# HBioquant/DiffBindFR

Hardware: AMD Instinct MI355X
Metric: poses_per_sec (higher is better)
Workload: dtype f32

## Files before the change

### diffbindfr_amd/build.py

```python
import os
import subprocess
import sys
from concurrent.futures import ThreadPoolExecutor

HERE = os.path.dirname(os.path.abspath(__file__))
CSRC = os.path.join(HERE, "csrc")
LIB = os.path.join(HERE, "libdbfr.so")
SOURCES = ["api.cpp", "so3_host.cpp", "conv.hip", "conv2.hip", "conv2h.hip", "convz.hip", "graph.hip", "heads.hip", "export.hip", "mdn.hip", "probe.hip", "vina.hip", "modes.hip", "posecheck.hip", "xtc.hip", "sites.hip", "interactions.hip", "pocketcheck.hip", "sasa.hip", "apoholo.hip", "hetero.hip"]
FLAGS = ["--offload-arch=gfx950", "-O3", "-std=c++17", "-fPIC", "-Wno-unused-result"]
if os.environ.get("DBFR_BUILD_DEV") == "1":
    FLAGS.append("-DDBFR_DEV_VARIANTS")
FILE_FLAGS = {"conv.hip": ["-ffp-contract=fast", "-fno-slp-vectorize", "-Wno-array-bounds"] + ([f"-DCONV_NB={os.environ['DBFR_BUILD_NB']}"] if "DBFR_BUILD_NB" in os.environ else [])
              + ([f"-DCONV_PRIO={os.environ['DBFR_BUILD_PRIO']}"] if "DBFR_BUILD_PRIO" in os.environ else [])
              + ([f"-DCONV_XPF={os.environ['DBFR_BUILD_XPF']}"] if "DBFR_BUILD_XPF" in os.environ else [])}
FILE_FLAGS["mdn.hip"] = ["-ffp-contract=off"]
FILE_FLAGS["conv2.hip"] = ["-ffp-contract=fast", "-fno-slp-vectorize", "-Wno-array-bounds"]
FILE_FLAGS["conv2h.hip"] = FILE_FLAGS["conv2.hip"] + ["-Rpass-analysis=kernel-resource-usage"]
FILE_FLAGS["convz.hip"] = FILE_FLAGS["conv2h.hip"]
DEFAULT_FP = ["-ffp-contract=off"]
FILE_FLAGS["vina.hip"] = DEFAULT_FP + ["-Rpass-analysis=kernel-resource-usage"]
FILE_FLAGS["modes.hip"] = FILE_FLAGS["vina.hip"]
FILE_FLAGS["posecheck.hip"] = FILE_FLAGS["vina.hip"]
FILE_FLAGS["xtc.hip"] = FILE_FLAGS["vina.hip"]
FILE_FLAGS["sites.hip"] = FILE_FLAGS["vina.hip"]
FILE_FLAGS["interactions.hip"] = FILE_FLAGS["vina.hip"]
FILE_FLAGS["pocketcheck.hip"] = FILE_FLAGS["vina.hip"]
FILE_FLAGS["sasa.hip"] = FILE_FLAGS["vina.hip"]
FILE_FLAGS["apoholo.hip"] = FILE_FLAGS["vina.hip"]
FILE_FLAGS["hetero.hip"] = FILE_FLAGS["vina.hip"]


def source_hash(dev=False):
    import hashlib
    h = hashlib.sha256()
    files = sorted([os.path.join(CSRC, f) for f in os.listdir(CSRC) if f.endswith((".cpp", ".hip", ".h", ".inc"))])
    files.append(os.path.join(HERE, "..", "include", "dbfr.h"))
    for f in files:
        h.update(os.path.basename(f).encode())
        h.update(open(f, "rb").read())
    if dev:
        h.update(b"DBFR_DEV_VARIANTS")
    return h.hexdigest()[:16]


def check_m0(hipcc, src):
    import re
    import tempfile
    with tempfile.TemporaryDirectory() as tmp:
        out = os.path.join(tmp, "convz.s")
        cmd = [hipcc, "-x", "hip", "-S", "--cuda-device-only", src, "-o", out] + [f for f in FLAGS + FILE_FLAGS["convz.hip"] if not f.startswith("-Rpass")]
        r = subprocess.run(cmd, capture_output=True, text=True)
        if r.returncode != 0:
            raise RuntimeError("hipcc -S failed (m0 check):\n" + r.stderr)
        lines = open(out).read().splitlines()
    ours = re.compile(r"^\s*s_mov_b32 m0, s\d+\s*$")
    bad = []
    for i, l in enumerate(lines):
        code = l.split(";")[0]
        if re.search(r"\bm0\b", code) and not ours.match(code):
            bad.append(f"{i + 1}: {l.strip()}")
        if ours.match(code) and not any("global_load_lds_dword" in x for x in lines[i + 1:i + 4]):
            bad.append(f"{i + 1}: s_mov_b32 m0 without an LDS-DMA load behind it: {l.strip()}")
    if bad:
        raise RuntimeError("convz.hip: the compiler (or an edit) uses m0 outside the LDS-DMA gathers -- the undeclared writes of prefetch_x are no longer safe:\n  " + "\n  ".join(bad[:10]))


def _stale(target, deps):
    if not os.path.exists(target):
        return True
    t = os.path.getmtime(target)
    return any(os.path.getmtime(d) > t for d in deps)


def build(force=False, verbose=True):
    hipcc = os.environ.get("HIPCC", "/opt/rocm/bin/hipcc")
    headers = [os.path.join(CSRC, "common.h"), os.path.join(CSRC, "frames.h"), os.path.join(CSRC, "residue_tables.inc"), os.path.join(HERE, "..", "include", "dbfr.h")]
    objs, jobs = [], []
    bid = source_hash(dev="-DDBFR_DEV_VARIANTS" in FLAGS)
    stamp = os.path.join(CSRC, ".build_id")
    if not os.path.exists(stamp) or open(stamp).read() != bid:
        open(stamp, "w").write(bid)
    headers.append(stamp)
# ... 29 lines not shown
```

### diffbindfr_amd/csrc/api.cpp

```cpp
#include <cmath>
#include <cstdio>
#include <cstring>
#include <algorithm>
#include <atomic>
#include <map>

#include "common.h"

void launch_conv(const ConvArgs& a, hipStream_t st);
void launch_conv_layer(const ConvArgs* c4, hipStream_t st);
void launch_conv2(const Conv2Args& a, hipStream_t st);
void launch_conv2h(const Conv2Args& a, hipStream_t st);
void launch_convz(const ConvZArgs& a, hipStream_t st);
void launch_reduce_ln(const float* msg, const int* row_start, const int* row_cnt, int N, int D, const LNDesc& ln,
                      const float* old, int D_old, float* out, int ldo, int mode, hipStream_t st, const uint8_t* first = nullptr, unsigned long long sc_lanes = 0);
struct ReduceLayerArgs {
  const float* msg[4]; const int* row_start[4]; const int* row_cnt[4]; LNDesc ln[4];
  int NL, NA, D, D_old;
  const float* old_l; const float* old_a; float* out_l; float* out_a;
  const uint8_t* first[4]; unsigned long long sc_lanes[4];
};
static unsigned long long convz_sc_lanes(const ConvZ& z) {
  unsigned long long m = 0;
  for (int i = 0; i < z.n_io; ++i) m |= 0xfffull << (z.out_off[i] / 4);
// ... 1633 lines not shown
  if (rc) return rc;
  if (!step || !scores || !z || !err_word_out) return fail(DBFR_ERR_ARG, "dbfr_test_sde_step: null argument");
  if (!scores->tr || !scores->rot || !z->z_tr || !z->z_rot || (b->NTOR > 0 && (!scores->tor || !z->z_tor)) ||
      (!m->cfg.no_sc_torsion && b->NSC > 0 && (!scores->sc_tor || !z->z_sc)))
    return fail(DBFR_ERR_ARG, "dbfr_test_sde_step: null score or noise array");
  hipStream_t st = (hipStream_t)hip_stream;
  HIPCHECK(hipMemsetAsync(err_word_out, 0, sizeof(int32_t), st));
  pose_update(m, b, *step, *scores, z->z_tr, z->z_rot, z->z_tor, z->z_sc, nullptr, atom14_out, nullptr, err_word_out, st);
  HIPCHECK(hipGetLastError());
  return DBFR_OK;
}

extern "C" int dbfr_test_chunk_table(const int32_t* tgt, const int32_t* n_edges_dev, int32_t max_edges, int32_t span, int32_t* scratch, int32_t cap,
                                     int32_t* chunk_es, int32_t* chunk_gl, void* hip_stream) {
  if (!tgt || !n_edges_dev || !scratch || !chunk_es || !chunk_gl || span <= 0 || max_edges < 0 || cap <= 0) return fail(DBFR_ERR_ARG, "dbfr_test_chunk_table: bad argument");
  g_launch_err = false;
  const int n_span = std::max((max_edges + span - 1) / span, 1);
  launch_flat_chunks(tgt, n_edges_dev, max_edges, span, n_span, scratch, cap, chunk_es, chunk_gl, (hipStream_t)hip_stream);
  HIPCHECK(hipGetLastError());
  return take_launch_error();
}

extern "C" int dbfr_test_conv(dbfr_model* m, int32_t layer, int32_t family, int32_t n_edges, const int32_t* n_edges_dev,
                              const int32_t* tgt, const int32_t* gth, const float* emb, const float* sh,
                              const float* tab1, int32_t ld1, const int32_t* idx1, const float* tab2, int32_t ld2,
                              const int32_t* idx2, const float* x, int32_t ldx, float* msg, void* hip_stream) {
  return test_conv_impl(m, false, layer, family, n_edges, n_edges_dev, tgt, gth, emb, sh, tab1, ld1, idx1, tab2, ld2, idx2, x, ldx,
                        msg, hip_stream);
}

extern "C" int dbfr_test_conv2(dbfr_model* m, int32_t layer, int32_t family, int32_t n_edges, const int32_t* n_edges_dev,
                               const int32_t* tgt, const int32_t* gth, const float* emb, const float* sh,
                               const float* tab1, int32_t ld1, const int32_t* idx1, const float* tab2, int32_t ld2,
                               const int32_t* idx2, const float* x, int32_t ldx, float* msg, void* hip_stream) {
  return test_conv_impl(m, true, layer, family, n_edges, n_edges_dev, tgt, gth, emb, sh, tab1, ld1, idx1, tab2, ld2, idx2, x, ldx,
                        msg, hip_stream);
}

extern "C" int dbfr_test_reduce_ln2(dbfr_model* m, int32_t layer, int32_t family, const float* msg, const int32_t* row_start, const int32_t* row_cnt,
                                    int32_t n_nodes, const float* old, int32_t d_old, float* out, int32_t mode, const uint8_t* seg_first, void* hip_stream) {
  if (!m) return fail(DBFR_ERR_ARG, "null model");
  const ConvW* cw = pick_conv(m, layer, family);
  if (!cw) return fail(DBFR_ERR_ARG, "no such conv");
  unsigned long long lanes = 0;
  if (seg_first) {
    if (layer == -1 || cw->K != 144) return fail(DBFR_ERR_ARG, "dbfr_test_reduce_ln2: seg_first with a conv that has no reduce-first form");
    lanes = convz_sc_lanes(layer >= 0 ? m->layerz[layer][family] : layer == -2 ? m->tor_convz : m->sc_convz);
  }
  launch_reduce_ln(msg, row_start, row_cnt, n_nodes, cw->D_out, cw->ln, old, d_old, out, cw->D_out, mode, (hipStream_t)hip_stream, seg_first, lanes);
  HIPCHECK(hipGetLastError());
  return DBFR_OK;
}

extern "C" int dbfr_test_reduce_ln(dbfr_model* m, int32_t layer, int32_t family, const float* msg,
                                   const int32_t* row_start, const int32_t* row_cnt, int32_t n_nodes, const float* old,
                                   int32_t d_old, float* out, int32_t mode, void* hip_stream) {
  if (!m) return fail(DBFR_ERR_ARG, "null model");
  const ConvW* cw = pick_conv(m, layer, family);
  if (!cw) return fail(DBFR_ERR_ARG, "no such conv");
  launch_reduce_ln(msg, row_start, row_cnt, n_nodes, cw->D_out, cw->ln, old, d_old, out, cw->D_out, mode,
                   (hipStream_t)hip_stream);
  HIPCHECK(hipGetLastError());
  return DBFR_OK;
}
```

### diffbindfr_amd/csrc/conv.hip

```cpp
#include <cstdio>
#include <cstdlib>
#include <type_traits>
#include <vector>

#include "common.h"

#ifndef CONV_PRIO
#define CONV_PRIO 0
#endif
#ifndef CONV_XPF
#define CONV_XPF 0
#endif
#ifndef CONV_NB2_WAVES
#define CONV_NB2_WAVES 2
#endif
#define XS_LD (MAXD + 4)

typedef float f32x4 __attribute__((ext_vector_type(4)));

#define TRACE_BLOCKS 1024
#define TRACE_TILES 48
#define TRACE_REC (2 + 3 * TRACE_TILES + 8)
#define RSTAMP(k) do { if ((ABL & 16) && a.trace && bid < TRACE_BLOCKS && lane == 0) a.trace[((size_t)bid * 4 + wave) * TRACE_REC + 2 + 3 * TRACE_TILES + (k)] = __builtin_amdgcn_s_memrealtime(); } while (0)
#define TSTAMP(k) do { if ((ABL & 16) && a.trace && bid < TRACE_BLOCKS && lane == 0) a.trace[((size_t)bid * 4 + wave) * TRACE_REC + 2 + 3 * TRACE_TILES + (k)] = __builtin_readcyclecounter(); } while (0)
// ... 462 lines not shown
  for (int bk = 0; bk < ln.nblk; ++bk) {
    const int mul = ln.mul[bk], dim = ln.dim[bk], off = ln.off[bk];
    const int nel = mul * dim;
    float mean[3] = {0.f, 0.f, 0.f};
    for (int i = lane; i < nel; i += 64) {
      int comp = i % dim;
      float v = buf[wave][off + i];
      if (comp == 0) mean[0] += v; else if (comp == 1) mean[1] += v; else mean[2] += v;
    }
#pragma unroll
    for (int c = 0; c < 3; ++c) {
      for (int o = 32; o > 0; o >>= 1) mean[c] += __shfl_xor(mean[c], o);
      mean[c] /= (float)mul;
    }
    float sq = 0.f;
    for (int i = lane; i < nel; i += 64) {
      int u = i / dim, comp = i - u * dim;
      float v = buf[wave][off + i] - (comp == 0 ? mean[0] : comp == 1 ? mean[1] : mean[2]) * ln.mean_shift[iw + u];
      buf[wave][off + i] = v;
      sq += v * v;
    }
    __syncthreads();
    for (int o = 32; o > 0; o >>= 1) sq += __shfl_xor(sq, o);
    const float inv = 1.0f / sqrtf(sq / (float)nel + 1e-5f);
    for (int i = lane; i < nel; i += 64) {
      int u = i / dim;
      float v = buf[wave][off + i] * (inv * ln.weight[iw + u]);
      if (ln.is0e[bk]) v += ln.bias[ib + u];
      buf[wave][off + i] = v;
    }
    iw += mul;
    if (ln.is0e[bk]) ib += mul;
  }
  __syncthreads();
#pragma unroll
  for (int j = 0; j < 3; ++j) {
    int c = lane + 64 * j;
    if (c < D && live) {
      float v = buf[wave][c];
      float* o = out + (size_t)node * ldo + c;
      if (mode == 0) v = (c < D_old ? old[(size_t)node * D_old + c] : 0.f) + v;
      else if (mode == 1) v = *o + v;
      *o = v;
    }
  }
}

void launch_reduce_ln(const float* msg, const int* row_start, const int* row_cnt, int N, int D, const LNDesc& ln,
                      const float* old, int D_old, float* out, int ldo, int mode, hipStream_t st, const uint8_t* first, unsigned long long sc_lanes) {
  if (N <= 0) return;
  hipLaunchKernelGGL(k_reduce_ln, dim3((N + 3) / 4), dim3(256), 0, st, msg, row_start, row_cnt, N, D, ln, old, D_old,
                     out, ldo, mode, first, sc_lanes);
}

struct ReduceLayerArgs {
  const float* msg[4]; const int* row_start[4]; const int* row_cnt[4]; LNDesc ln[4];
  int NL, NA, D, D_old;
  const float* old_l; const float* old_a; float* out_l; float* out_a;
  const uint8_t* first[4]; unsigned long long sc_lanes[4];
};

__device__ __forceinline__ void mean_ln(const float* __restrict__ msg, int rs, int rc, int D, const LNDesc& ln, float* bw, int lane, const uint8_t* first, unsigned long long sc_lanes) {
  const int d4 = D >> 2;
  const f32x4 acc = row_sum(msg, rs, rc, D, lane, first, sc_lanes);
  if (lane < d4) {
    const float cntf = (float)max(rc, 1);
    bw[4 * lane] = acc[0] / cntf; bw[4 * lane + 1] = acc[1] / cntf; bw[4 * lane + 2] = acc[2] / cntf; bw[4 * lane + 3] = acc[3] / cntf;
  }
  __builtin_amdgcn_wave_barrier();
  int iw = 0, ib = 0;
  for (int bk = 0; bk < ln.nblk; ++bk) {
    const int mul = ln.mul[bk], dim = ln.dim[bk], off = ln.off[bk];
    const int nel = mul * dim;
    float mean[3] = {0.f, 0.f, 0.f};
    const bool d3 = dim == 3;
    for (int i = lane; i < nel; i += 64) {
      int comp = d3 ? i % 3 : 0;
      float v = bw[off + i];
      if (comp == 0) mean[0] += v; else if (comp == 1) mean[1] += v; else mean[2] += v;
    }
    for (int o = 32; o > 0; o >>= 1) mean[0] += __shfl_xor(mean[0], o);
    mean[0] /= (float)mul;
    if (d3) {
#pragma unroll
      for (int c = 1; c < 3; ++c) {
        for (int o = 32; o > 0; o >>= 1) mean[c] += __shfl_xor(mean[c], o);
        mean[c] /= (float)mul;
      }
    }
    float sq = 0.f;
    for (int i = lane; i < nel; i += 64) {
      int u = d3 ? i / 3 : i, comp = d3 ? i - 3 * u : 0;
      float v = bw[off + i] - (comp == 0 ? mean[0] : comp == 1 ? mean[1] : mean[2]) * ln.mean_shift[iw + u];
      bw[off + i] = v;
      sq += v * v;
    }
    __builtin_amdgcn_wave_barrier();
    for (int o = 32; o > 0; o >>= 1) sq += __shfl_xor(sq, o);
    const float inv = 1.0f / sqrtf(sq / (float)nel + 1e-5f);
    for (int i = lane; i < nel; i += 64) {
      int u = d3 ? i / 3 : i;
      float v = bw[off + i] * (inv * ln.weight[iw + u]);
      if (ln.is0e[bk]) v += ln.bias[ib + u];
      bw[off + i] = v;
    }
    iw += mul;
    if (ln.is0e[bk]) ib += mul;
  }
  __builtin_amdgcn_wave_barrier();
}

__global__ __launch_bounds__(256) void k_reduce_ln_layer(ReduceLayerArgs a) {
  __shared__ float buf[4][2][MAXD];
  const int lane = threadIdx.x & 63, wave = threadIdx.x >> 6;
  const int nbl = (a.NL + 3) / 4;
  const bool lig = (int)blockIdx.x < nbl;
  const int node = (lig ? blockIdx.x : blockIdx.x - nbl) * 4 + wave;
  const int N = lig ? a.NL : a.NA;
  if (node >= N) return;
  const int s0 = lig ? 0 : 2;
  mean_ln(a.msg[s0], a.row_start[s0][node], a.row_cnt[s0][node], a.D, a.ln[s0], buf[wave][0], lane, a.first[s0], a.sc_lanes[s0]);
  mean_ln(a.msg[s0 + 1], a.row_start[s0 + 1][node], a.row_cnt[s0 + 1][node], a.D, a.ln[s0 + 1], buf[wave][1], lane, a.first[s0 + 1], a.sc_lanes[s0 + 1]);
  const float* old = (lig ? a.old_l : a.old_a) + (size_t)node * a.D_old;
  float* out = (lig ? a.out_l : a.out_a) + (size_t)node * a.D;
#pragma unroll
  for (int j = 0; j < 3; ++j) {
    const int c = lane + 64 * j;
    if (c < a.D) out[c] = ((c < a.D_old ? old[c] : 0.f) + buf[wave][0][c]) + buf[wave][1][c];
  }
}

void launch_reduce_ln_layer(const ReduceLayerArgs& a, hipStream_t st) {
  const int nb = (a.NL + 3) / 4 + (a.NA + 3) / 4;
  if (nb <= 0) return;
  hipLaunchKernelGGL(k_reduce_ln_layer, dim3(nb), dim3(256), 0, st, a);
}
```

### diffbindfr_amd/lib.py

```python
import ctypes as C
import os

HERE = os.path.dirname(os.path.abspath(__file__))
LIB_PATH = os.environ.get("DBFR_LIB") or os.path.join(HERE, "libdbfr.so")

DBFR_OK = 0
DBFR_ERR_CAPACITY = -3
ERRORS = {-1: "DBFR_ERR_ARG", -2: "DBFR_ERR_HIP", -3: "DBFR_ERR_CAPACITY", -4: "DBFR_ERR_SELFTEST",
          -5: "DBFR_ERR_NUMERIC"}

i32, f32, vp = C.c_int32, C.c_float, C.c_void_p


class ModelCfg(C.Structure):
    _fields_ = [(n, i32) for n in ("ns", "nv", "sh_lmax", "num_conv_layers", "lig_node_features",
                                   "lig_edge_features", "distance_embed_dim", "sigma_embed_dim")] + \
               [(n, f32) for n in ("emb_scale", "lig_cutoff", "atom_cutoff", "cross_cutoff", "center_max_distance")] + \
               [(n, i32) for n in ("atom_max_neighbors", "lig_max_neighbors", "dynamic_max_cross", "scale_by_sigma",
                                   "no_sc_torsion")]


class Tensor(C.Structure):
    _fields_ = [("name", C.c_char_p), ("data", vp), ("numel", C.c_int64)]

# ... 179 lines not shown


class HeteroCheckIn(C.Structure):
    _fields_ = [("n_group", C.c_int32), ("n_frame", C.c_int32)] + \
               [(n, C.c_void_p) for n in ("frame_ptr", "lig_ptr", "lig_pos_off", "lig_pos", "lig_rad", "lig_cov", "lig_flags", "het_ptr",
                                          "het_pos", "het_rad", "het_cov", "het_class", "het_metal", "pocket_ptr", "pocket_pos_off",
                                          "pocket_pos", "pocket_polar", "pocket_col", "static_ptr", "static_pos", "static_polar",
                                          "static_col", "res_ptr")] + \
               [(n, C.c_int32) for n in ("max_lig", "max_pocket", "max_res", "cand_cap")] + [("host", C.c_void_p)]


class HeteroCheckOpts(C.Structure):
    _fields_ = [(n, C.c_float) for n in ("clash_ratio", "displace_dist", "metal_dist", "hbond_dist", "grid")] + \
               [("vol_scale", C.c_float * 3), ("vol_overlap_max", C.c_float * 3), ("max_event", C.c_int32)]


class HeteroCheckOut(C.Structure):
    _fields_ = [(n, C.c_void_p) for n in ("min_dist", "min_ratio", "worst", "n_clash", "vol_lig", "vol_overlap", "n_displaced", "n_bridge",
                                          "n_coord", "passed", "event_i", "event_f", "n_event")]


class PdbLigand(C.Structure):
    _fields_ = [("n_atoms", i32), ("head", C.c_char_p), ("atom_line", C.POINTER(C.c_char_p)), ("tail", C.c_char_p)]


class XtcIn(C.Structure):
    _fields_ = [(n, i32) for n in ("n_frame", "n_file", "n_src", "n_lig", "n_res", "n_static", "n_map", "max_atoms")] + \
               [(n, vp) for n in ("lig", "pos14", "center", "static_pos", "map_ptr", "atom_map", "file_map", "frame_file",
                                  "frame_src", "frame_step")]


class XtcOpts(C.Structure):
    _fields_ = [("precision", f32), ("dt", f32), ("first_step", i32), ("box", f32 * 9)]


class SitesOpts(C.Structure):
    _fields_ = [(n, f32) for n in ("spacing", "probe", "ray_length", "lining_cutoff")] + \
               [(n, i32) for n in ("min_buried", "min_points", "max_sites")]


class SitesIn(C.Structure):
    _fields_ = [("n_prot", i32), ("n_res", i32), ("max_points", C.c_int64)] + \
               [(n, vp) for n in ("res_ptr", "aatype", "atom37_pos", "atom37_mask", "radius")]


class SitesOut(C.Structure):
    _fields_ = [(n, vp) for n in ("n_sites", "label", "n_points", "score", "idx_sum", "centre", "lining", "grid", "occupancy",
                                  "burial", "labels")]


SYMBOLS = ["dbfr_model_create", "dbfr_model_destroy", "dbfr_model_set_edge_log", "dbfr_model_set_tie_log", "dbfr_model_fallback_convs", "dbfr_model_rowscaled_convs", "dbfr_model_set_gemm", "dbfr_model_get_gemm", "dbfr_workspace_bytes", "dbfr_score", "dbfr_sample",
           "dbfr_sample_range", "dbfr_capacity_report",
           "dbfr_init_poses", "dbfr_extract_templates", "dbfr_status_sync", "dbfr_abi_version", "dbfr_build_id", "dbfr_last_error", "dbfr_wigner3j", "dbfr_conv_paths", "dbfr_test_pack_f16_tiles", "dbfr_test_pack_f16_rows", "dbfr_test_chunk_table", "dbfr_test_pack_f16_depth", "dbfr_probe_mfma_f16",
           "dbfr_profile_enable", "dbfr_profile_read", "dbfr_profile_fused_bytes", "dbfr_profile_executed_flops", "dbfr_profile_useful_flops", "dbfr_workspace_layout", "dbfr_test_conv", "dbfr_test_conv2", "dbfr_test_reduce_ln", "dbfr_test_reduce_ln2", "dbfr_test_sde_step",
           "dbfr_pose_metrics", "dbfr_pdb_format", "dbfr_pdb_write_files", "dbfr_select_pocket", "dbfr_sdf_format",
           "dbfr_sdf_write_files", "dbfr_mdn_model_create", "dbfr_mdn_model_destroy", "dbfr_mdn_workspace_bytes", "dbfr_mdn_forward", "dbfr_mdn_pocket_features",
           "dbfr_vina_workspace_bytes", "dbfr_vina_score", "dbfr_vina_score_at", "dbfr_vina_minimize",
           "dbfr_pose_rmsd_matrix", "dbfr_select_modes", "dbfr_pose_check",
           "dbfr_pdb_atom_map", "dbfr_complex_pdb_format", "dbfr_complex_pdb_write_files", "dbfr_xtc_workspace_bytes", "dbfr_xtc_encode",
           "dbfr_sites_workspace_bytes", "dbfr_find_sites", "dbfr_interactions", "dbfr_pocket_check", "dbfr_sasa",
           "dbfr_seq_align", "dbfr_holo_site", "dbfr_holo_metrics", "dbfr_hetero_check"]

_lib = None


class DbfrError(RuntimeError):
    pass


def load():
    global _lib
    if _lib is not None:
        return _lib
    if not os.path.exists(LIB_PATH):
        raise DbfrError(f"{LIB_PATH} is missing: build the HIP library first "
                        f"(python -m diffbindfr_amd.build). There is no CPU fallback.")
    lib = C.CDLL(LIB_PATH)
    lib.dbfr_last_error.restype = C.c_char_p
    lib.dbfr_build_id.restype = C.c_char_p
    lib.dbfr_model_create.argtypes = [C.POINTER(ModelCfg), C.POINTER(Tensor), i32, C.POINTER(vp)]
    lib.dbfr_model_destroy.argtypes = [vp]
    lib.dbfr_model_destroy.restype = None
    lib.dbfr_model_set_edge_log.argtypes = [vp, vp, i32, i32]
    lib.dbfr_model_set_tie_log.argtypes = [vp, vp, i32, i32, C.c_float]
    lib.dbfr_model_fallback_convs.argtypes = [vp, C.c_char_p, C.c_size_t]
    lib.dbfr_model_rowscaled_convs.argtypes = [vp, C.c_char_p, C.c_size_t]
    lib.dbfr_model_set_gemm.argtypes = [vp, i32]
    lib.dbfr_model_get_gemm.argtypes = [vp]
    lib.dbfr_workspace_bytes.argtypes = [vp, C.POINTER(Batch), C.POINTER(Limits), C.POINTER(C.c_size_t)]
    lib.dbfr_score.argtypes = [vp, C.POINTER(Batch), C.POINTER(Cond), C.POINTER(Scores), vp, C.c_size_t,
                               C.POINTER(Limits), vp]
    lib.dbfr_sample.argtypes = [vp, C.POINTER(Batch), C.POINTER(Step), i32, C.POINTER(Noise), vp, vp, vp, vp,
                                C.c_size_t, C.POINTER(Limits), vp]
    lib.dbfr_sample_range.argtypes = [vp, C.POINTER(Batch), C.POINTER(Step), i32, i32, C.POINTER(Noise), vp, vp, vp, vp,
                                      C.c_size_t, C.POINTER(Limits), vp]
    lib.dbfr_capacity_report.argtypes = [vp, vp, C.POINTER(i32), C.POINTER(C.c_int64)]
    lib.dbfr_init_poses.argtypes = [vp, C.POINTER(Batch), C.POINTER(InitTape), vp, vp]
    lib.dbfr_extract_templates.argtypes = [i32, vp, vp, vp, vp, vp, vp, vp, vp]
    lib.dbfr_status_sync.argtypes = [vp, vp, C.POINTER(C.c_int64)]
    lib.dbfr_wigner3j.argtypes = [i32, i32, i32, C.POINTER(C.c_double)]
    lib.dbfr_conv_paths.argtypes = [i32, C.POINTER(i32), i32, C.POINTER(i32)]
    lib.dbfr_test_pack_f16_tiles.argtypes = [vp, vp, i32, vp, C.POINTER(i32)]
    lib.dbfr_test_pack_f16_depth.argtypes = [vp, vp, i32, C.POINTER(i32), C.POINTER(i32)]
    lib.dbfr_test_pack_f16_rows.argtypes = [vp, vp, i32, vp, C.POINTER(i32), vp, C.POINTER(i32)]
    lib.dbfr_test_chunk_table.argtypes = [vp, vp, i32, i32, vp, i32, vp, vp, vp]
    lib.dbfr_probe_mfma_f16.argtypes = [C.c_double, C.POINTER(C.c_double), vp]
    lib.dbfr_profile_enable.argtypes = [vp, i32]
    lib.dbfr_profile_fused_bytes.argtypes = [vp, C.POINTER(C.c_double)]
    lib.dbfr_profile_executed_flops.argtypes = [vp, C.POINTER(C.c_double)]
    lib.dbfr_profile_useful_flops.argtypes = [vp, C.POINTER(C.c_double), C.POINTER(C.c_double)]
    lib.dbfr_profile_read.argtypes = [vp, C.POINTER(C.c_double), C.POINTER(C.c_int64), C.POINTER(C.c_double),
                                      C.POINTER(C.c_double), i32]
    lib.dbfr_workspace_layout.argtypes = [vp, C.POINTER(Batch), C.POINTER(Limits), C.c_char_p, C.c_size_t,
                                          C.POINTER(C.c_size_t), C.POINTER(C.c_size_t), i32]
    lib.dbfr_test_conv.argtypes = [vp, i32, i32, i32, vp, vp, vp, vp, vp, vp, i32, vp, vp, i32, vp, vp, i32, vp, vp]
    lib.dbfr_test_conv2.argtypes = lib.dbfr_test_conv.argtypes
    lib.dbfr_test_reduce_ln.argtypes = [vp, i32, i32, vp, vp, vp, i32, vp, i32, vp, i32, vp]
    lib.dbfr_test_reduce_ln2.argtypes = [vp, i32, i32, vp, vp, vp, i32, vp, i32, vp, i32, vp, vp]
    lib.dbfr_test_sde_step.argtypes = [vp, C.POINTER(Batch), C.POINTER(Step), C.POINTER(Scores), C.POINTER(Noise), vp, vp, vp]
    lib.dbfr_select_pocket.argtypes = [i32, i32, vp, i32, vp, vp, vp, vp, C.c_double, i32, vp, vp, vp]
    lib.dbfr_pose_metrics.argtypes = [C.POINTER(PoseMetricsIn), C.POINTER(PoseMetricsOut), vp]
    lib.dbfr_pdb_format.argtypes = [C.POINTER(PdbTopology), i32, vp, vp, i32, i32, vp, C.c_int64]
    lib.dbfr_pdb_format.restype = C.c_int64
    lib.dbfr_pdb_write_files.argtypes = [C.POINTER(PdbTopology), i32, vp, vp, i32, C.POINTER(C.c_char_p), i32]
    lib.dbfr_sdf_format.argtypes = [C.POINTER(SdfTemplate), vp, vp, C.c_int64]
    lib.dbfr_sdf_format.restype = C.c_int64
    lib.dbfr_sdf_write_files.argtypes = [C.POINTER(SdfTemplate), vp, i32, C.POINTER(C.c_char_p), i32]
    lib.dbfr_mdn_model_create.argtypes = [C.POINTER(Tensor), i32, C.POINTER(vp)]
    lib.dbfr_mdn_model_destroy.argtypes = [vp]
    lib.dbfr_mdn_model_destroy.restype = None
    lib.dbfr_mdn_workspace_bytes.argtypes = [C.POINTER(MdnBatch), C.POINTER(C.c_size_t)]
    lib.dbfr_mdn_pocket_features.argtypes = [i32, i32, vp, vp, vp, vp, i32, vp, vp, vp, vp, vp, vp, vp, vp]
    lib.dbfr_mdn_forward.argtypes = [vp, C.POINTER(MdnBatch), vp, vp, vp, vp, C.c_size_t, vp]
    lib.dbfr_vina_workspace_bytes.argtypes = [C.POINTER(VinaIn), C.POINTER(C.c_size_t)]
    lib.dbfr_vina_score.argtypes = [C.POINTER(VinaIn), vp, vp, vp, vp, C.c_size_t, vp]
    lib.dbfr_vina_score_at.argtypes = [C.POINTER(VinaIn), vp, vp, vp, vp, vp, vp, vp, C.c_size_t, vp]
    lib.dbfr_vina_minimize.argtypes = [C.POINTER(VinaIn), C.POINTER(VinaOpts), vp, vp, vp, vp, C.c_size_t, vp]
    lib.dbfr_pose_rmsd_matrix.argtypes = [C.POINTER(PoseRmsdIn), vp, vp]
    lib.dbfr_select_modes.argtypes = [C.POINTER(PoseRmsdIn), vp, vp, C.POINTER(ModesOpts), vp, vp, vp, vp]
    lib.dbfr_pose_check.argtypes = [C.POINTER(PoseCheckIn), C.POINTER(PoseCheckOpts), C.POINTER(PoseCheckOut), vp]
    lib.dbfr_pdb_atom_map.argtypes = [C.POINTER(PdbTopology), i32, vp, vp, vp, C.c_int64, C.POINTER(C.c_int64)]
    lib.dbfr_pdb_atom_map.restype = C.c_int64
    lib.dbfr_complex_pdb_format.argtypes = [C.POINTER(PdbTopology), i32, vp, vp, C.POINTER(PdbLigand), vp, vp, C.c_int64]
    lib.dbfr_complex_pdb_format.restype = C.c_int64
    lib.dbfr_complex_pdb_write_files.argtypes = [C.POINTER(PdbTopology), i32, vp, vp, C.POINTER(PdbLigand), vp, i32,
                                                 C.POINTER(C.c_char_p), i32]
    lib.dbfr_xtc_workspace_bytes.argtypes = [C.POINTER(XtcIn), C.POINTER(C.c_size_t), C.POINTER(C.c_int64)]
    lib.dbfr_xtc_encode.argtypes = [C.POINTER(XtcIn), C.POINTER(XtcOpts), vp, C.c_int64, vp, vp, C.c_size_t, vp]
    lib.dbfr_sites_workspace_bytes.argtypes = [C.POINTER(SitesIn), C.POINTER(C.c_size_t)]
    lib.dbfr_find_sites.argtypes = [C.POINTER(SitesIn), C.POINTER(SitesOpts), C.POINTER(SitesOut), vp, C.c_size_t, vp]
    lib.dbfr_interactions.argtypes = [C.POINTER(InteractionsIn), C.POINTER(InteractionsOpts), C.POINTER(InteractionsOut), vp]
    lib.dbfr_pocket_check.argtypes = [C.POINTER(PocketCheckIn), C.POINTER(PocketCheckOpts), C.POINTER(PocketCheckOut), vp]
    lib.dbfr_sasa.argtypes = [C.POINTER(SasaIn), C.POINTER(SasaOpts), C.POINTER(SasaOut), vp]
    lib.dbfr_seq_align.argtypes = [i32, vp, vp, vp, vp, vp, vp, i32]
    lib.dbfr_holo_site.argtypes = [C.POINTER(HoloSiteIn), vp, vp]
    lib.dbfr_holo_metrics.argtypes = [C.POINTER(HoloMetricsIn), C.POINTER(HoloMetricsOpts), C.POINTER(HoloMetricsOut), vp]
    lib.dbfr_hetero_check.argtypes = [C.POINTER(HeteroCheckIn), C.POINTER(HeteroCheckOpts), C.POINTER(HeteroCheckOut), vp]
    if lib.dbfr_abi_version() != 7:
        raise DbfrError("libdbfr ABI version mismatch")
    _lib = lib
    return lib


def check(rc):
    if rc != DBFR_OK:
        msg = load().dbfr_last_error().decode()
        raise DbfrError(f"{ERRORS.get(rc, rc)}: {msg}")


def workspace_views(model_handle, batch_c, limits, ws):
    lib = load()
# ... 11 lines not shown
```

### include/dbfr.h

```cpp
#ifndef DBFR_H
#define DBFR_H

#include <stddef.h>
#include <stdint.h>

#ifdef __cplusplus
extern "C" {
#endif

#define DBFR_ABI_VERSION 7

typedef enum {
  DBFR_OK = 0,
  DBFR_ERR_ARG = -1,
  DBFR_ERR_HIP = -2,
  DBFR_ERR_CAPACITY = -3,
  DBFR_ERR_SELFTEST = -4,
  DBFR_ERR_NUMERIC = -5
} dbfr_status;

typedef struct dbfr_model dbfr_model;

typedef struct {
  int32_t ns, nv, sh_lmax;
// ... 700 lines not shown

int dbfr_sites_workspace_bytes(const dbfr_sites_in* in, size_t* bytes);
int dbfr_find_sites(const dbfr_sites_in* in, const dbfr_sites_opts* opts, const dbfr_sites_out* out, void* workspace,
                    size_t workspace_bytes, void* hip_stream);

int dbfr_status_sync(void* workspace, void* hip_stream, int64_t* counters);

#define DBFR_GEMM_F32 0
#define DBFR_GEMM_SPLIT_F16 3
#define DBFR_GEMM_REDUCE_FIRST 4
#define DBFR_GEMM_DEFAULT DBFR_GEMM_REDUCE_FIRST
int dbfr_model_set_gemm(dbfr_model* model, int32_t mode);
int dbfr_model_rowscaled_convs(const dbfr_model* model, char* names, size_t names_cap);
int dbfr_model_fallback_convs(const dbfr_model* model, char* names, size_t names_cap);
int dbfr_model_get_gemm(const dbfr_model* model);

int         dbfr_abi_version(void);
const char* dbfr_build_id(void);
const char* dbfr_last_error(void);
int dbfr_wigner3j(int32_t l1, int32_t l2, int32_t l3, double* out);
int dbfr_conv_paths(int32_t kind, int32_t* table10, int32_t max_paths, int32_t* weight_numel);
int dbfr_test_chunk_table(const int32_t* tgt, const int32_t* n_edges_dev, int32_t max_edges, int32_t span, int32_t* scratch, int32_t cap,
                          int32_t* chunk_es, int32_t* chunk_gl, void* hip_stream);
int dbfr_test_pack_f16_tiles(const float* frag, const float* bias, int32_t n_tiles, void* out, int32_t* k_out);
int dbfr_test_pack_f16_rows(const float* frag, const float* bias, int32_t n_tiles, void* out, int32_t* k_out, float* rinv_out, int32_t* depth_out);
int dbfr_test_pack_f16_depth(const float* frag, const float* bias, int32_t n_tiles, int32_t* depth_out, int32_t* depth_ok_out);
int dbfr_profile_enable(dbfr_model* m, int32_t on);
int dbfr_profile_read(dbfr_model* m, double* conv_ms, int64_t* conv_launches, double* conv_flops,
                      double* ref_form_bytes, int32_t reset);
int dbfr_profile_fused_bytes(const dbfr_model* m, double* fused_form_bytes);
int dbfr_profile_executed_flops(const dbfr_model* m, double* executed_flops);
int dbfr_profile_useful_flops(const dbfr_model* m, double* useful_flops, double* form_bytes);

int dbfr_probe_mfma_f16(double seconds, double* tflops, void* hip_stream);

int dbfr_workspace_layout(const dbfr_model* m, const dbfr_batch* b, const dbfr_limits* lim, char* names,
                          size_t names_cap, size_t* offsets, size_t* bytes, int32_t max_entries);

int dbfr_test_conv(dbfr_model* m, int32_t layer, int32_t family, int32_t n_edges, const int32_t* n_edges_dev,
                   const int32_t* tgt, const int32_t* gth, const float* emb, const float* sh, const float* tab1,
                   int32_t ld1, const int32_t* idx1, const float* tab2, int32_t ld2, const int32_t* idx2,
                   const float* x, int32_t ldx, float* msg, void* hip_stream);
int dbfr_test_conv2(dbfr_model* m, int32_t layer, int32_t family, int32_t n_edges, const int32_t* n_edges_dev,
                    const int32_t* tgt, const int32_t* gth, const float* emb, const float* sh, const float* tab1,
                    int32_t ld1, const int32_t* idx1, const float* tab2, int32_t ld2, const int32_t* idx2,
                    const float* x, int32_t ldx, float* msg, void* hip_stream);
int dbfr_test_reduce_ln(dbfr_model* m, int32_t layer, int32_t family, const float* msg, const int32_t* row_start,
                        const int32_t* row_cnt, int32_t n_nodes, const float* old, int32_t d_old, float* out,
                        int32_t mode, void* hip_stream);
int dbfr_test_reduce_ln2(dbfr_model* m, int32_t layer, int32_t family, const float* msg, const int32_t* row_start,
                         const int32_t* row_cnt, int32_t n_nodes, const float* old, int32_t d_old, float* out,
                         int32_t mode, const uint8_t* seg_first, void* hip_stream);

int dbfr_test_sde_step(const dbfr_model* m, const dbfr_batch* b, const dbfr_step* step, const dbfr_scores* scores,
                       const dbfr_noise* z, float* atom14_out, int32_t* err_word_out, void* hip_stream);

#ifdef __cplusplus
}
#endif
#endif
```

Measured before the change: 521.1.

## Rewrite layer reduce+LayerNorm kernel with register-resident params and butterfly reductions

Moves the per-layer mean-aggregation plus equivariant LayerNorm kernel into its own file and restructures it. LN parameters live in registers per block, and both message families are processed together as float2 pairs. Block means and variances use ds_bpermute butterflies instead of repeated LDS loops and shuffles, and the segment sum is unrolled by 8 with ballot-based first-flag masking. The aim is fewer LDS round trips, serial loops and barriers. In exchange the kernel only accepts irreps layouts with at most 4 blocks of up to 64 elements and rejects others at launch.

```diff
diff --git a/diffbindfr_amd/build.py b/diffbindfr_amd/build.py
--- a/diffbindfr_amd/build.py
+++ b/diffbindfr_amd/build.py
@@ -6,7 +6,7 @@
 HERE = os.path.dirname(os.path.abspath(__file__))
 CSRC = os.path.join(HERE, "csrc")
 LIB = os.path.join(HERE, "libdbfr.so")
-SOURCES = ["api.cpp", "so3_host.cpp", "conv.hip", "conv2.hip", "conv2h.hip", "convz.hip", "graph.hip", "heads.hip", "export.hip", "mdn.hip", "probe.hip", "vina.hip", "modes.hip", "posecheck.hip", "xtc.hip", "sites.hip", "interactions.hip", "pocketcheck.hip", "sasa.hip", "apoholo.hip", "hetero.hip"]
+SOURCES = ["api.cpp", "so3_host.cpp", "conv.hip", "conv2.hip", "conv2h.hip", "convz.hip", "graph.hip", "heads.hip", "export.hip", "mdn.hip", "probe.hip", "vina.hip", "modes.hip", "posecheck.hip", "xtc.hip", "sites.hip", "interactions.hip", "pocketcheck.hip", "sasa.hip", "apoholo.hip", "hetero.hip", "reduce.hip"]
 FLAGS = ["--offload-arch=gfx950", "-O3", "-std=c++17", "-fPIC", "-Wno-unused-result"]
 if os.environ.get("DBFR_BUILD_DEV") == "1":
     FLAGS.append("-DDBFR_DEV_VARIANTS")
@@ -28,6 +28,7 @@
 FILE_FLAGS["sasa.hip"] = FILE_FLAGS["vina.hip"]
 FILE_FLAGS["apoholo.hip"] = FILE_FLAGS["vina.hip"]
 FILE_FLAGS["hetero.hip"] = FILE_FLAGS["vina.hip"]
+FILE_FLAGS["reduce.hip"] = FILE_FLAGS["vina.hip"]
 
 
 def source_hash(dev=False):
diff --git a/diffbindfr_amd/csrc/api.cpp b/diffbindfr_amd/csrc/api.cpp
--- a/diffbindfr_amd/csrc/api.cpp
+++ b/diffbindfr_amd/csrc/api.cpp
@@ -1709,6 +1709,25 @@
   return DBFR_OK;
 }
 
+extern "C" int dbfr_test_reduce_ln_layer(dbfr_model* m, int32_t layer, const float* const* msg, const int32_t* const* row_start, const int32_t* const* row_cnt,
+                                         const uint8_t* const* seg_first, const float* old_l, const float* old_a, int32_t n_lig, int32_t n_atom,
+                                         float* out_l, float* out_a, void* hip_stream) {
+  if (!m) return fail(DBFR_ERR_ARG, "null model");
+  if (layer < 0 || layer >= m->cfg.num_conv_layers) return fail(DBFR_ERR_ARG, "dbfr_test_reduce_ln_layer: no such layer");
+  if (!msg || !row_start || !row_cnt || !seg_first || n_lig < 0 || n_atom < 0) return fail(DBFR_ERR_ARG, "dbfr_test_reduce_ln_layer: bad argument");
+  static const int dims[4] = {48, 84, 120, 168};
+  ReduceLayerArgs ra;
+  for (int i = 0; i < 4; ++i) {
+    ra.msg[i] = msg[i]; ra.row_start[i] = row_start[i]; ra.row_cnt[i] = row_cnt[i]; ra.ln[i] = m->layer[layer][i].ln;
+    ra.first[i] = seg_first[i]; ra.sc_lanes[i] = seg_first[i] ? convz_sc_lanes(m->layerz[layer][i]) : 0;
+  }
+  ra.NL = n_lig; ra.NA = n_atom; ra.D = dims[std::min(layer + 1, 3)]; ra.D_old = dims[std::min(layer, 3)];
+  ra.old_l = old_l; ra.old_a = old_a; ra.out_l = out_l; ra.out_a = out_a;
+  launch_reduce_ln_layer(ra, (hipStream_t)hip_stream);
+  HIPCHECK(hipGetLastError());
+  return DBFR_OK;
+}
+
 extern "C" int dbfr_test_reduce_ln(dbfr_model* m, int32_t layer, int32_t family, const float* msg,
                                    const int32_t* row_start, const int32_t* row_cnt, int32_t n_nodes, const float* old,
                                    int32_t d_old, float* out, int32_t mode, void* hip_stream) {
diff --git a/diffbindfr_amd/csrc/conv.hip b/diffbindfr_amd/csrc/conv.hip
--- a/diffbindfr_amd/csrc/conv.hip
+++ b/diffbindfr_amd/csrc/conv.hip
@@ -538,86 +538,3 @@
   hipLaunchKernelGGL(k_reduce_ln, dim3((N + 3) / 4), dim3(256), 0, st, msg, row_start, row_cnt, N, D, ln, old, D_old,
                      out, ldo, mode, first, sc_lanes);
 }
-
-struct ReduceLayerArgs {
-  const float* msg[4]; const int* row_start[4]; const int* row_cnt[4]; LNDesc ln[4];
-  int NL, NA, D, D_old;
-  const float* old_l; const float* old_a; float* out_l; float* out_a;
-  const uint8_t* first[4]; unsigned long long sc_lanes[4];
-};
-
-__device__ __forceinline__ void mean_ln(const float* __restrict__ msg, int rs, int rc, int D, const LNDesc& ln, float* bw, int lane, const uint8_t* first, unsigned long long sc_lanes) {
-  const int d4 = D >> 2;
-  const f32x4 acc = row_sum(msg, rs, rc, D, lane, first, sc_lanes);
-  if (lane < d4) {
-    const float cntf = (float)max(rc, 1);
-    bw[4 * lane] = acc[0] / cntf; bw[4 * lane + 1] = acc[1] / cntf; bw[4 * lane + 2] = acc[2] / cntf; bw[4 * lane + 3] = acc[3] / cntf;
-  }
-  __builtin_amdgcn_wave_barrier();
-  int iw = 0, ib = 0;
-  for (int bk = 0; bk < ln.nblk; ++bk) {
-    const int mul = ln.mul[bk], dim = ln.dim[bk], off = ln.off[bk];
-    const int nel = mul * dim;
-    float mean[3] = {0.f, 0.f, 0.f};
-    const bool d3 = dim == 3;
-    for (int i = lane; i < nel; i += 64) {
-      int comp = d3 ? i % 3 : 0;
-      float v = bw[off + i];
-      if (comp == 0) mean[0] += v; else if (comp == 1) mean[1] += v; else mean[2] += v;
-    }
-    for (int o = 32; o > 0; o >>= 1) mean[0] += __shfl_xor(mean[0], o);
-    mean[0] /= (float)mul;
-    if (d3) {
-#pragma unroll
-      for (int c = 1; c < 3; ++c) {
-        for (int o = 32; o > 0; o >>= 1) mean[c] += __shfl_xor(mean[c], o);
-        mean[c] /= (float)mul;
-      }
-    }
-    float sq = 0.f;
-    for (int i = lane; i < nel; i += 64) {
-      int u = d3 ? i / 3 : i, comp = d3 ? i - 3 * u : 0;
-      float v = bw[off + i] - (comp == 0 ? mean[0] : comp == 1 ? mean[1] : mean[2]) * ln.mean_shift[iw + u];
-      bw[off + i] = v;
-      sq += v * v;
-    }
-    __builtin_amdgcn_wave_barrier();
-    for (int o = 32; o > 0; o >>= 1) sq += __shfl_xor(sq, o);
-    const float inv = 1.0f / sqrtf(sq / (float)nel + 1e-5f);
-    for (int i = lane; i < nel; i += 64) {
-      int u = d3 ? i / 3 : i;
-      float v = bw[off + i] * (inv * ln.weight[iw + u]);
-      if (ln.is0e[bk]) v += ln.bias[ib + u];
-      bw[off + i] = v;
-    }
-    iw += mul;
-    if (ln.is0e[bk]) ib += mul;
-  }
-  __builtin_amdgcn_wave_barrier();
-}
-
-__global__ __launch_bounds__(256) void k_reduce_ln_layer(ReduceLayerArgs a) {
-  __shared__ float buf[4][2][MAXD];
-  const int lane = threadIdx.x & 63, wave = threadIdx.x >> 6;
-  const int nbl = (a.NL + 3) / 4;
-  const bool lig = (int)blockIdx.x < nbl;
-  const int node = (lig ? blockIdx.x : blockIdx.x - nbl) * 4 + wave;
-  const int N = lig ? a.NL : a.NA;
-  if (node >= N) return;
-  const int s0 = lig ? 0 : 2;
-  mean_ln(a.msg[s0], a.row_start[s0][node], a.row_cnt[s0][node], a.D, a.ln[s0], buf[wave][0], lane, a.first[s0], a.sc_lanes[s0]);
-  mean_ln(a.msg[s0 + 1], a.row_start[s0 + 1][node], a.row_cnt[s0 + 1][node], a.D, a.ln[s0 + 1], buf[wave][1], lane, a.first[s0 + 1], a.sc_lanes[s0 + 1]);
-  const float* old = (lig ? a.old_l : a.old_a) + (size_t)node * a.D_old;
-  float* out = (lig ? a.out_l : a.out_a) + (size_t)node * a.D;
-#pragma unroll
-  for (int j = 0; j < 3; ++j) {
-    const int c = lane + 64 * j;
-    if (c < a.D) out[c] = ((c < a.D_old ? old[c] : 0.f) + buf[wave][0][c]) + buf[wave][1][c];
-  }
-}
-
-void launch_reduce_ln_layer(const ReduceLayerArgs& a, hipStream_t st) {
-  const int nb = (a.NL + 3) / 4 + (a.NA + 3) / 4;
-  if (nb <= 0) return;
-  hipLaunchKernelGGL(k_reduce_ln_layer, dim3(nb), dim3(256), 0, st, a);
-}
diff --git a/diffbindfr_amd/csrc/reduce.hip b/diffbindfr_amd/csrc/reduce.hip
--- /dev/null
+++ b/diffbindfr_amd/csrc/reduce.hip
@@ -0,0 +1,187 @@
+#include "common.h"
+
+typedef float f32x4 __attribute__((ext_vector_type(4)));
+typedef float f32x2 __attribute__((ext_vector_type(2)));
+
+struct ReduceLayerArgs {
+  const float* msg[4]; const int* row_start[4]; const int* row_cnt[4]; LNDesc ln[4];
+  int NL, NA, D, D_old;
+  const float* old_l; const float* old_a; float* out_l; float* out_a;
+  const uint8_t* first[4]; unsigned long long sc_lanes[4];
+};
+
+#define RL_MAXBLK 4
+
+template <bool FLAG>
+__device__ __forceinline__ f32x4 seg_sum(const f32x4* __restrict__ r, int d4, int rc, bool ld, bool sc, const uint8_t* __restrict__ first, int lane) {
+  f32x4 acc = {0.f, 0.f, 0.f, 0.f};
+  const f32x4 zero = {0.f, 0.f, 0.f, 0.f};
+  for (int e0 = 0; e0 < rc; e0 += 64) {
+    const int nb = min(64, rc - e0);
+    unsigned long long fl = ~0ull;
+    if (FLAG) fl = __ballot(lane < nb && first[e0 + lane] != 0);
+    if (ld) {
+      const f32x4* p = r + (size_t)e0 * d4;
+      auto take = [&](int i) { return !FLAG || !sc || ((fl >> i) & 1ull); };
+      auto row = [&](int i) { return take(i) ? p[(size_t)i * d4] : zero; };
+      int e = 0;
+      for (; e + 8 <= nb; e += 8) {
+        const f32x4 v0 = row(e), v1 = row(e + 1), v2 = row(e + 2), v3 = row(e + 3), v4 = row(e + 4), v5 = row(e + 5), v6 = row(e + 6), v7 = row(e + 7);
+        acc += v0; acc += v1; acc += v2; acc += v3; acc += v4; acc += v5; acc += v6; acc += v7;
+      }
+      for (; e + 4 <= nb; e += 4) {
+        const f32x4 v0 = row(e), v1 = row(e + 1), v2 = row(e + 2), v3 = row(e + 3);
+        acc += v0; acc += v1; acc += v2; acc += v3;
+      }
+      for (; e < nb; ++e)
+        if (take(e)) acc += p[(size_t)e * d4];
+    }
+  }
+  return acc;
+}
+
+__device__ __forceinline__ f32x2 bfly(f32x2 v, const int (&xa)[6]) {
+#pragma unroll
+  for (int k = 0; k < 6; ++k) {
+    f32x2 o;
+    o.x = __int_as_float(__builtin_amdgcn_ds_bpermute(xa[k], __float_as_int(v.x)));
+    o.y = __int_as_float(__builtin_amdgcn_ds_bpermute(xa[k], __float_as_int(v.y)));
+    v += o;
+  }
+  return v;
+}
+
+__global__ __launch_bounds__(256) void k_reduce_ln_layer(ReduceLayerArgs a) {
+  __shared__ __attribute__((aligned(16))) float buf[4][2][MAXD];
+  const int lane = threadIdx.x & 63, wave = __builtin_amdgcn_readfirstlane(threadIdx.x >> 6);
+  const int nbl = (a.NL + 3) / 4;
+  const bool lig = (int)blockIdx.x < nbl;
+  const int N = lig ? a.NL : a.NA;
+  const int node = (lig ? blockIdx.x : blockIdx.x - nbl) * 4 + wave;
+  if (node >= N) return;
+  const int s0 = lig ? 0 : 2;
+  const LNDesc& lnA = a.ln[s0];
+  const LNDesc& lnB = a.ln[s0 + 1];
+  const int D = a.D, d4 = D >> 2, D_old = a.D_old;
+  const float* msgA = a.msg[s0];
+  const float* msgB = a.msg[s0 + 1];
+  const int *rsA = a.row_start[s0], *rcA = a.row_cnt[s0], *rsB = a.row_start[s0 + 1], *rcB = a.row_cnt[s0 + 1];
+  const uint8_t *fA = a.first[s0], *fB = a.first[s0 + 1];
+  const bool scA = (a.sc_lanes[s0] >> lane) & 1ull, scB = (a.sc_lanes[s0 + 1] >> lane) & 1ull;
+  const float* oldp = lig ? a.old_l : a.old_a;
+  float* outp = lig ? a.out_l : a.out_a;
+  const bool ld = lane < d4;
+  const int lc = min(lane, d4 - 1);
+  int xa[6];
+#pragma unroll
+  for (int k = 0; k < 6; ++k) xa[k] = (lane ^ (32 >> k)) << 2;
+  const int l3 = lane / 3, c3 = lane - 3 * l3;
+  const int nblk = lnA.nblk;
+  int off[RL_MAXBLK], iw0[RL_MAXBLK], ib0[RL_MAXBLK];
+  bool act[RL_MAXBLK], d3[RL_MAXBLK], is0e[RL_MAXBLK];
+  float mulf[RL_MAXBLK];
+  f32x2 sh[RL_MAXBLK], wt[RL_MAXBLK], bi[RL_MAXBLK];
+  float nelf = 1.f;
+  {
+    int iw = 0, ib = 0;
+#pragma unroll
+    for (int bk = 0; bk < RL_MAXBLK; ++bk) {
+      off[bk] = 0; iw0[bk] = 0; ib0[bk] = 0; act[bk] = false; d3[bk] = false; is0e[bk] = false; mulf[bk] = 1.f;
+      sh[bk] = f32x2{0.f, 0.f}; wt[bk] = f32x2{0.f, 0.f}; bi[bk] = f32x2{0.f, 0.f};
+      if (bk < nblk) {
+        const int mul = lnA.mul[bk], dim = lnA.dim[bk], nel = mul * dim;
+        d3[bk] = dim == 3;
+        is0e[bk] = lnA.is0e[bk] != 0;
+        act[bk] = lane < nel;
+        off[bk] = lnA.off[bk]; iw0[bk] = iw; ib0[bk] = ib;
+        mulf[bk] = (float)mul;
+        if ((lane & 3) == bk) nelf = (float)nel;
+        iw += mul;
+        if (is0e[bk]) ib += mul;
+      }
+    }
+  }
+  auto load_params = [&]() {
+#pragma unroll
+    for (int bk = 0; bk < RL_MAXBLK; ++bk)
+      if (act[bk]) {
+        const int u = d3[bk] ? l3 : lane, pw = iw0[bk] + u, pb = ib0[bk] + u;
+        sh[bk] = f32x2{lnA.mean_shift[pw], lnB.mean_shift[pw]};
+        wt[bk] = f32x2{lnA.weight[pw], lnB.weight[pw]};
+        if (is0e[bk]) bi[bk] = f32x2{lnA.bias[pb], lnB.bias[pb]};
+      }
+  };
+  float* bwA = buf[wave][0];
+  float* bwB = buf[wave][1];
+  {
+    const int ra = rsA[node], ca = rcA[node], rb = rsB[node], cb = rcB[node];
+    float oldv[RL_MAXBLK];
+#pragma unroll
+    for (int bk = 0; bk < RL_MAXBLK; ++bk) oldv[bk] = (act[bk] && (off[bk] + lane) < D_old) ? oldp[(size_t)node * D_old + (off[bk] + lane)] : 0.f;
+    const f32x4* pa = reinterpret_cast<const f32x4*>(msgA + (size_t)ra * D) + lc;
+    const f32x4* pb = reinterpret_cast<const f32x4*>(msgB + (size_t)rb * D) + lc;
+    const f32x4 sa = fA ? seg_sum<true>(pa, d4, ca, ld, scA, fA + ra, lane) : seg_sum<false>(pa, d4, ca, ld, false, nullptr, lane);
+    const f32x4 sb = fB ? seg_sum<true>(pb, d4, cb, ld, scB, fB + rb, lane) : seg_sum<false>(pb, d4, cb, ld, false, nullptr, lane);
+    load_params();
+    if (ld) {
+      const float fa = (float)max(ca, 1), fb = (float)max(cb, 1);
+      *reinterpret_cast<f32x4*>(bwA + 4 * lane) = f32x4{sa[0] / fa, sa[1] / fa, sa[2] / fa, sa[3] / fa};
+      *reinterpret_cast<f32x4*>(bwB + 4 * lane) = f32x4{sb[0] / fb, sb[1] / fb, sb[2] / fb, sb[3] / fb};
+    }
+    __builtin_amdgcn_wave_barrier();
+    f32x2 v[RL_MAXBLK], sq[RL_MAXBLK];
+#pragma unroll
+    for (int bk = 0; bk < RL_MAXBLK; ++bk) {
+      v[bk] = f32x2{0.f, 0.f}; sq[bk] = f32x2{0.f, 0.f};
+      if (bk < nblk) {
+        const f32x2 zero = {0.f, 0.f};
+        const f32x2 x = act[bk] ? f32x2{bwA[(off[bk] + lane)], bwB[(off[bk] + lane)]} : zero;
+        const f32x2 x0 = zero + x;
+        f32x2 m = bfly((act[bk] && (!d3[bk] || c3 == 0)) ? x0 : zero, xa);
+        if (d3[bk]) {
+          const f32x2 m1 = bfly((act[bk] && c3 == 1) ? x0 : zero, xa);
+          const f32x2 m2 = bfly((act[bk] && c3 == 2) ? x0 : zero, xa);
+          m = c3 == 0 ? m : c3 == 1 ? m1 : m2;
+        }
+        m.x = m.x / mulf[bk]; m.y = m.y / mulf[bk];
+        f32x2 s = zero;
+        if (act[bk]) {
+          v[bk] = f32x2{__builtin_fmaf(-sh[bk].x, m.x, x.x), __builtin_fmaf(-sh[bk].y, m.y, x.y)};
+          s = f32x2{__builtin_fmaf(v[bk].x, v[bk].x, 0.f), __builtin_fmaf(v[bk].y, v[bk].y, 0.f)};
+        }
+        sq[bk] = bfly(s, xa);
+      }
+    }
+    float t = sq[0].x;
+    t = (lane & 7) == 1 ? sq[1].x : t; t = (lane & 7) == 2 ? sq[2].x : t; t = (lane & 7) == 3 ? sq[3].x : t;
+    t = (lane & 7) == 4 ? sq[0].y : t; t = (lane & 7) == 5 ? sq[1].y : t; t = (lane & 7) == 6 ? sq[2].y : t; t = (lane & 7) == 7 ? sq[3].y : t;
+    t = 1.0f / sqrtf(t / nelf + 1e-5f);
+    float* o = outp + (size_t)node * D;
+#pragma unroll
+    for (int bk = 0; bk < RL_MAXBLK; ++bk) {
+      if (bk < nblk) {
+        const float ia = __int_as_float(__builtin_amdgcn_readlane(__float_as_int(t), bk));
+        const float ib = __int_as_float(__builtin_amdgcn_readlane(__float_as_int(t), 4 + bk));
+        float ya = v[bk].x * (ia * wt[bk].x), yb = v[bk].y * (ib * wt[bk].y);
+        if (is0e[bk]) { ya = ya + bi[bk].x; yb = yb + bi[bk].y; }
+        if (act[bk]) o[(off[bk] + lane)] = (oldv[bk] + ya) + yb;
+      }
+    }
+  }
+}
+
+void launch_reduce_ln_layer(const ReduceLayerArgs& a, hipStream_t st) {
+  const int nb = (a.NL + 3) / 4 + (a.NA + 3) / 4;
+  if (nb <= 0) return;
+  bool ok = a.D > 0 && a.D <= MAXD && (a.D & 3) == 0 && a.ln[0].nblk >= 1 && a.ln[0].nblk <= RL_MAXBLK;
+  for (int i = 0; ok && i < 4; ++i) {
+    ok = a.ln[i].nblk == a.ln[0].nblk;
+    for (int bk = 0; ok && bk < a.ln[i].nblk; ++bk) {
+      const int dim = a.ln[i].dim[bk], nel = a.ln[i].mul[bk] * dim;
+      ok = (dim == 1 || dim == 3) && nel >= 1 && nel <= 64 && a.ln[i].off[bk] >= 0 && a.ln[i].off[bk] + nel <= a.D && a.ln[i].mul[bk] == a.ln[0].mul[bk] &&
+           dim == a.ln[0].dim[bk] && a.ln[i].off[bk] == a.ln[0].off[bk] && (a.ln[i].is0e[bk] != 0) == (a.ln[0].is0e[bk] != 0);
+    }
+  }
+  if (dbfr_launch_check(ok ? hipSuccess : hipErrorInvalidValue, "launch_reduce_ln_layer: out irreps the layer reduction has no layout for")) return;
+  hipLaunchKernelGGL(k_reduce_ln_layer, dim3(nb), dim3(256), 0, st, a);
+}
diff --git a/diffbindfr_amd/lib.py b/diffbindfr_amd/lib.py
--- a/diffbindfr_amd/lib.py
+++ b/diffbindfr_amd/lib.py
@@ -255,7 +255,7 @@
 SYMBOLS = ["dbfr_model_create", "dbfr_model_destroy", "dbfr_model_set_edge_log", "dbfr_model_set_tie_log", "dbfr_model_fallback_convs", "dbfr_model_rowscaled_convs", "dbfr_model_set_gemm", "dbfr_model_get_gemm", "dbfr_workspace_bytes", "dbfr_score", "dbfr_sample",
            "dbfr_sample_range", "dbfr_capacity_report",
            "dbfr_init_poses", "dbfr_extract_templates", "dbfr_status_sync", "dbfr_abi_version", "dbfr_build_id", "dbfr_last_error", "dbfr_wigner3j", "dbfr_conv_paths", "dbfr_test_pack_f16_tiles", "dbfr_test_pack_f16_rows", "dbfr_test_chunk_table", "dbfr_test_pack_f16_depth", "dbfr_probe_mfma_f16",
-           "dbfr_profile_enable", "dbfr_profile_read", "dbfr_profile_fused_bytes", "dbfr_profile_executed_flops", "dbfr_profile_useful_flops", "dbfr_workspace_layout", "dbfr_test_conv", "dbfr_test_conv2", "dbfr_test_reduce_ln", "dbfr_test_reduce_ln2", "dbfr_test_sde_step",
+           "dbfr_profile_enable", "dbfr_profile_read", "dbfr_profile_fused_bytes", "dbfr_profile_executed_flops", "dbfr_profile_useful_flops", "dbfr_workspace_layout", "dbfr_test_conv", "dbfr_test_conv2", "dbfr_test_reduce_ln", "dbfr_test_reduce_ln2", "dbfr_test_reduce_ln_layer", "dbfr_test_sde_step",
            "dbfr_pose_metrics", "dbfr_pdb_format", "dbfr_pdb_write_files", "dbfr_select_pocket", "dbfr_sdf_format",
            "dbfr_sdf_write_files", "dbfr_mdn_model_create", "dbfr_mdn_model_destroy", "dbfr_mdn_workspace_bytes", "dbfr_mdn_forward", "dbfr_mdn_pocket_features",
            "dbfr_vina_workspace_bytes", "dbfr_vina_score", "dbfr_vina_score_at", "dbfr_vina_minimize",
@@ -320,6 +320,7 @@
     lib.dbfr_test_conv2.argtypes = lib.dbfr_test_conv.argtypes
     lib.dbfr_test_reduce_ln.argtypes = [vp, i32, i32, vp, vp, vp, i32, vp, i32, vp, i32, vp]
     lib.dbfr_test_reduce_ln2.argtypes = [vp, i32, i32, vp, vp, vp, i32, vp, i32, vp, i32, vp, vp]
+    lib.dbfr_test_reduce_ln_layer.argtypes = [vp, i32, C.POINTER(vp), C.POINTER(vp), C.POINTER(vp), C.POINTER(vp), vp, vp, i32, i32, vp, vp, vp]
     lib.dbfr_test_sde_step.argtypes = [vp, C.POINTER(Batch), C.POINTER(Step), C.POINTER(Scores), C.POINTER(Noise), vp, vp, vp]
     lib.dbfr_select_pocket.argtypes = [i32, i32, vp, i32, vp, vp, vp, vp, C.c_double, i32, vp, vp, vp]
     lib.dbfr_pose_metrics.argtypes = [C.POINTER(PoseMetricsIn), C.POINTER(PoseMetricsOut), vp]
diff --git a/include/dbfr.h b/include/dbfr.h
--- a/include/dbfr.h
+++ b/include/dbfr.h
@@ -776,6 +776,10 @@
                          const int32_t* row_cnt, int32_t n_nodes, const float* old, int32_t d_old, float* out,
                          int32_t mode, const uint8_t* seg_first, void* hip_stream);
 
+int dbfr_test_reduce_ln_layer(dbfr_model* m, int32_t layer, const float* const* msg, const int32_t* const* row_start,
+                              const int32_t* const* row_cnt, const uint8_t* const* seg_first, const float* old_l, const float* old_a,
+                              int32_t n_lig, int32_t n_atom, float* out_l, float* out_a, void* hip_stream);
+
 int dbfr_test_sde_step(const dbfr_model* m, const dbfr_batch* b, const dbfr_step* step, const dbfr_scores* scores,
                        const dbfr_noise* z, float* atom14_out, int32_t* err_word_out, void* hip_stream);
 
```

New measurement: 526.0, median of 6. About the same (+0.9%).
